# reesque/SfmFromScratch

Measured on AMD Instinct MI355X. Metric: images/sec detect+describe+match, 1080p, 1/2/4/8 MI355X, higher is better.
Workload: dtype f32; 1 GPU; BASELINE configs[1]: 32x 1080p per GPU, ScaleRotInvSIFT 4-level x2 octave pyramid, k=2500, fw 18, NNRatio 0.85 over consecutive pairs; frames_per_gpu=32, pairs_per_gpu=31, distinct_batches=2, parallelism=image-shard x1, batches_in_flight=2

## Files before the change

include/sfmfeat.h:

```cpp
#ifndef SFMFEAT_H_
#define SFMFEAT_H_

#include <stddef.h>
#include <stdint.h>

#ifdef __cplusplus
extern "C" {
#endif

#define SFM_OK 0
#define SFM_EINVAL 1
#define SFM_ESTATE 2
#define SFM_EDEVICE 3
#define SFM_ERANGE 4
#define SFM_EINDEX 5

#define SFM_MODE_SCALEROT 0
#define SFM_MODE_NAIVE 1

#define SFM_DESC_DIM 128
#define SFM_MAX_GAUSS 15
#define SFM_MAX_KSIZE 31
#define SFM_MAX_FW 64
#define SFM_MAX_LEVELS 12
// ... 158 lines not shown
#define SFM_PROF_MEDIAN 2
#define SFM_PROF_NMS 3
#define SFM_PROF_TOPK 4
#define SFM_PROF_DESCRIBE 5
#define SFM_PROF_MATCH_PREP 6
#define SFM_PROF_MATCH 7
#define SFM_PROF_MATCH_POST 8
#define SFM_PROF_STAGES 9
int32_t sfm_profile_enable(sfm_ctx* ctx, int32_t on);
int32_t sfm_profile_stages(sfm_ctx* ctx, int32_t mask);
int32_t sfm_profile_read(sfm_ctx* ctx, double* ms, int64_t* launches, int32_t reset);
int32_t sfm_profile_spans(sfm_ctx* ctx, int64_t capacity);
int32_t sfm_profile_spans_read(sfm_ctx* ctx, int64_t* spans_ns, int32_t* levels, int64_t cap, int64_t* n_out,
                               int64_t* dropped, int32_t reset);

int32_t sfm_debug_atan2(int32_t device, const float* y, const float* x, float* out, int64_t n);
int32_t sfm_debug_harris(int32_t device, const float* gauss, int32_t gs, double alpha,
                         int32_t ksize, const float* img, int32_t H, int32_t W, float* R_out,
                         float* median_out, int64_t* ncand_out);

int32_t sfm_debug_nms(int32_t device, const float* R, int32_t B, int32_t H, int32_t W, int32_t ksize,
                      const uint32_t* tnms, int32_t tile, uint64_t* keys_out, int64_t* counts_out);

float sfm_debug_time_harris(int32_t device, int32_t abl, int32_t B, int32_t H, int32_t W,
                            int32_t iters);
float sfm_debug_harris_stamps(int32_t device, int32_t abl, int32_t B, int32_t H, int32_t W,
                              int32_t iters, uint64_t* out, int64_t cap);

int64_t sfm_debug_match_stamps(uint64_t* out, int64_t cap);

int32_t sfm_copy_wg(void* dst, const void* src, int64_t bytes, int32_t workgroups, void* stream);

int32_t sfm_debug_select_stats(sfm_ctx* ctx, int32_t* fallback_planes, int32_t* total_planes);
int32_t sfm_debug_pose_candidates(sfm_ctx* ctx, int32_t* cand_idx, int64_t entries);
int32_t sfm_debug_copy_level(sfm_ctx* ctx, int32_t l, int32_t what, float* out, void* stream);


#ifdef __cplusplus
}
#endif

#endif
```

sfmfromscratch_amd/_native.py:

```python
from __future__ import annotations

import ctypes
import os
import sys
import threading

import numpy as np

from . import _abi
from ._abi import SfmParams

_HERE = os.path.dirname(os.path.abspath(__file__))
LIB_PATH = os.environ.get("SFMFEAT_LIB", os.path.join(_HERE, "lib", "libsfmfeat.so"))

_lib = None
_lib_lock = threading.Lock()

_fp = ctypes.POINTER(ctypes.c_float)
_i64p = ctypes.POINTER(ctypes.c_int64)
_i32p = ctypes.POINTER(ctypes.c_int32)
_u8p = ctypes.POINTER(ctypes.c_uint8)
_dp = ctypes.POINTER(ctypes.c_double)
_vp = ctypes.c_void_p

# ... 68 lines not shown
    "sfm_profile_read": (ctypes.c_int32, [_vp, ctypes.POINTER(ctypes.c_double), _i64p, ctypes.c_int32]),
    "sfm_profile_spans": (ctypes.c_int32, [_vp, ctypes.c_int64]),
    "sfm_profile_spans_read": (ctypes.c_int32, [_vp, _i64p, _i32p, ctypes.c_int64, _i64p, _i64p, ctypes.c_int32]),
    "sfm_debug_time_harris": (ctypes.c_float, [ctypes.c_int32] * 6),
    "sfm_debug_harris_stamps": (ctypes.c_float, [ctypes.c_int32] * 6 + [ctypes.c_void_p, ctypes.c_int64]),
    "sfm_debug_match_stamps": (ctypes.c_int64, [ctypes.c_void_p, ctypes.c_int64]),
    "sfm_debug_select_stats": (ctypes.c_int32, [_vp, _i32p, _i32p]),
    "sfm_copy_wg": (ctypes.c_int32, [_vp, _vp, ctypes.c_int64, ctypes.c_int32, _vp]),
    "sfm_dist_unique_id": (ctypes.c_int32, [_u8p]),
    "sfm_dist_create": (ctypes.c_int32, [ctypes.c_int32, ctypes.c_int32, ctypes.c_int32, _u8p, ctypes.POINTER(_vp)]),
    "sfm_dist_destroy": (ctypes.c_int32, [_vp]),
    "sfm_dist_last_error": (ctypes.c_char_p, [_vp]),
    "sfm_dist_rank": (ctypes.c_int32, [_vp, _i32p, _i32p]),
    "sfm_dist_allgather_slots_dev": (ctypes.c_int32, [_vp, ctypes.c_int32, ctypes.c_int32, _vp, _vp, _vp, _vp, _vp,
                                                      _vp, ctypes.c_int64, _vp]),
    "sfm_dist_halo_dev": (ctypes.c_int32, [_vp, ctypes.c_int32, _vp, _vp, _vp, _vp, _vp, _vp, _vp]),

    "sfm_debug_copy_level": (ctypes.c_int32, [_vp, ctypes.c_int32, ctypes.c_int32, _vp, _vp]),
    "sfm_debug_atan2": (ctypes.c_int32, [ctypes.c_int32, _fp, _fp, _fp, ctypes.c_int64]),
    "sfm_debug_harris": (ctypes.c_int32, [ctypes.c_int32, _fp, ctypes.c_int32, ctypes.c_double, ctypes.c_int32,
                                          _fp, ctypes.c_int32, ctypes.c_int32, _fp, _fp, _i64p]),
    "sfm_debug_nms": (ctypes.c_int32, [ctypes.c_int32, _fp, ctypes.c_int32, ctypes.c_int32, ctypes.c_int32,
                                       ctypes.c_int32, _vp, ctypes.c_int32, _vp, _i64p]),
}


class NativeLibraryMissing(ImportError):
    pass


def _preload_torch_hip_runtime():
    import importlib.util
    spec = importlib.util.find_spec("torch")
    if spec is None or not spec.submodule_search_locations:
        return
    for d in spec.submodule_search_locations:
        cand = os.path.join(d, "lib", "libamdhip64.so")
        if os.path.exists(cand):
            try:
                ctypes.CDLL(cand, mode=ctypes.RTLD_GLOBAL)
            except OSError:
                pass
            return


def _preload_torch_rccl():
# ... 281 lines not shown
    H, W = img.shape
    gs = int(params.gaussian_size)
    g = np.array(params.gauss_kernel[: gs * gs], np.float32)
    R = np.empty_like(img)
    med = np.zeros(1, np.float32)
    nc = ctypes.c_int64(0)
    check(load_library().sfm_debug_harris(device, g.ctypes.data_as(_fp), gs, params.alpha, params.ksize,
                                          img.ctypes.data_as(_fp), H, W, R.ctypes.data_as(_fp),
                                          med.ctypes.data_as(_fp), ctypes.byref(nc)))
    return R, med[0], nc.value


def debug_nms(R: np.ndarray, tnms, ksize: int = 3, tile: bool = False, device: int = 0):
    R = np.ascontiguousarray(R, dtype=np.float32)
    B, H, W = R.shape
    t = np.ascontiguousarray(tnms, dtype=np.uint32)
    keys = np.zeros(B * H * W, np.uint64)
    cnt = np.zeros(B, np.int64)
    check(load_library().sfm_debug_nms(device, R.ctypes.data_as(_fp), B, H, W, ksize, t.ctypes.data,
                                       int(tile), keys.ctypes.data, cnt.ctypes.data_as(_i64p)))
    return [np.sort(keys[b * H * W: b * H * W + cnt[b]]) for b in range(B)]


class Gate:

    def __init__(self, device: int = 0):
        self.lib = load_library()
        h = _vp()
        if self.lib.sfm_gate_create(device, ctypes.byref(h)) != _abi.SFM_OK:
            raise RuntimeError("sfm_gate_create failed: no usable MI355X (HIP) device")
        self.handle = h

    def attach(self, ctx: Context):
        check(self.lib.sfm_ctx_set_gate(ctx.handle, self.handle), ctx.handle)

    def close(self):
        if getattr(self, "handle", None) is not None and self.handle.value:
            self.lib.sfm_gate_destroy(self.handle)
            self.handle = _vp()

    def __del__(self):
        try:
            self.close()
        except Exception:
            pass

# ... 85 lines not shown
```

sfmfromscratch_amd/csrc/api_extract.hip:

```cpp
#include "ctx.h"

using namespace sfm;

static_assert(kLayoutMedBins == kMedBins1 && kLayoutCounterStride == kCounterStride &&
                  kLayoutMedianStateBytes == sizeof(MedianState) && kLayoutSelectMaxLevels == kSelectMaxLevels,
              "extract_layout.h mirrors kernels.h");

const ExtractSwitches& extract_switches() {
  static const ExtractSwitches sw = [] {
    ExtractSwitches s;
    s.layout.pyr_fused = env_int(getenv("SFMFEAT_PYR_FUSED"), 1) != 0;
    s.layout.exact_px = env_int(getenv("SFMFEAT_EXACT_PX"), 128);
    s.layout.select_merge = env_int(SFM_DIAG_ENV("SFMFEAT_SELECT_MERGE"), 1) != 0;
    s.fill_launches = env_int(SFM_DIAG_ENV("SFMFEAT_FILL_LAUNCHES"), 0) != 0;
    s.harris_group = env_int(SFM_DIAG_ENV("SFMFEAT_HARRIS_GROUP"), 0);
    s.gate_level = env_int(SFM_DIAG_ENV("SFMFEAT_GATE_LEVEL"), 0);
    s.select_caller = env_int(SFM_DIAG_ENV("SFMFEAT_SELECT_CALLER"), 0) == 1;
    s.skip = env_int(SFM_ABLATION_ENV("SFMFEAT_SKIP"), 0);
    return s;
  }();
  return sw;
}

namespace {
// ... 104 lines not shown
    g.n = y.L - y.L_aux;
    for (int l = y.L_aux; l < y.L; ++l)
      g.l[l - y.L_aux] = SelectLevels::Level{R(l), cand(l), candcnt + y.counter[l], at<uint32_t>(kBufMedlist, y.sel[l]),
                                             at<uint64_t>(kBufScratch, y.sel[l]), kp(l), med(l), y.lv[l].h, y.lv[l].w,
                                             y.lv[l].fw / 2};
    if (!(skip & 1)) launch_select_levels(g, std::max(c->kcap, 1), c->kcap, B, c->p.ksize, st);
  }

  void describe_level(int l, hipStream_t s) {
    StageScope sc(c, SFM_PROF_DESCRIBE, s);
    const int L = y.L;
    if ((skip & 2) && l != L - 1) {
      fused_ok = false;
      return;
    }
    bool ow = false;
    const bool r = launch_describe(lvl[l], B, y.lv[l].h, y.lv[l].w, y.lv[l].fw, c->p.mode == SFM_MODE_NAIVE ? 0 : 1,
                                   kp(l), c->kcap, as<int32_t>(c->ex.buf[kBufLc]), l, L, y.lv[l].scale, xy, desc, conf,
                                   cap, l == L - 1 ? count : nullptr, mo, &ow, s);
    if (l == L - 1) counted = r;
    fused_ok = fused_ok && ow;
  }

  int release_gate() {
    if (c->gate && !gate_released) {
      HIPCHK(c, hipEventRecord(c->gate->ev, st));
      c->gate->armed = true;
      gate_released = true;
    }
    return SFM_OK;
  }

  int run(const float* imgs);
};

int Extraction::run(const float* imgs) {
  const int L = y.L, L_aux = y.L_aux;
  CtxStreams& cs = c->s;
  int rc;
  lvl[0] = imgs;
  for (int l = 1; l < L; ++l) lvl[l] = at<float>(kBufLvl, y.lvl[l]);
  zeroed = sw.fill_launches;
  {
    StageScope sc(c, SFM_PROF_PYRAMID, st);
    if (!y.pyr_fused) pyramid_from(1);
  }
// ... 27 lines not shown
    for (int l = l0; l < l1; ++l) {
      if (!exact(l)) {
        StageScope sc(c, SFM_PROF_NMS, st);
        launch_nms(R(l), med(l), cand(l), candcnt + y.counter[l], B, y.lv[l].h, y.lv[l].w, c->p.ksize, 0, st);
      }
      if (l < L_aux) {
        if (sw.select_caller) select_level(l, st);
        HIPCHK(c, hipEventRecord(cs.ev[l], st));
        HIPCHK(c, hipStreamWaitEvent(ax, cs.ev[l], 0));
        if (!sw.select_caller) select_level(l, ax);
        if (l == L_aux - 1) HIPCHK(c, hipEventRecord(cs.ev[L + 2], ax));
        describe_level(l, ax);
      }
    }
    l0 = l1;
  }
  if ((rc = release_gate())) return rc;
  if (y.select_merged) {
    select_merged();
  } else {
    for (int l = L_aux; l < L; ++l) select_level(l, st);
  }
  if (L_aux > 0 && L > L_aux) HIPCHK(c, hipStreamWaitEvent(st, cs.ev[L + 2], 0));
  for (int l = L_aux; l < L; ++l) describe_level(l, st);
  if (L_aux > 0) {
    HIPCHK(c, hipEventRecord(cs.ev[L + 1], ax));
    HIPCHK(c, hipStreamWaitEvent(st, cs.ev[L + 1], 0));
  }
  if (!counted) launch_finalize_counts(as<int32_t>(c->ex.buf[kBufLc]), B, L, count, st);
  HIPCHK(c, hipGetLastError());
  if (fused_ok && counted) operands_fused_commit(c, B);
  return SFM_OK;
}

}

int extract_reserve(sfm_ctx* c, int B, int H, int W) {
  ExtractLayout y;
  if (int rc = layout_of(c, B, H, W, &y)) return rc;
  return reserve(c, y);
}

int extract_impl(sfm_ctx* c, const float* imgs, int B, int H, int W, int32_t* xy, float* desc, float* conf,
                 int32_t* count, int64_t cap, hipStream_t st) {
  if (B < 1 || H < 1 || W < 1) return set_err(c, SFM_EINVAL, "empty batch or image");
  if (cap < c->cap) return set_err(c, SFM_ERANGE, "slot capacity below L * int(k / L)");
  ExtractLayout y;
// ... 88 lines not shown
```

sfmfromscratch_amd/csrc/debug.hip:

```cpp
#include <string.h>

#include <vector>

#include "../../include/sfmfeat.h"
#include "kernels.h"

using namespace sfm;

namespace sfm {

__global__ void k_debug_atan2(const float* __restrict__ y, const float* __restrict__ x,
                              float* __restrict__ out, int64_t n) {
  int64_t i = (int64_t)blockIdx.x * blockDim.x + threadIdx.x;
  if (i < n) out[i] = svml_atan2f(y[i], x[i]);
}

__global__ void __launch_bounds__(256) k_copy_wg(const uint4* __restrict__ src, uint4* __restrict__ dst, int64_t n16,
                                                 const uint8_t* __restrict__ src_b, uint8_t* __restrict__ dst_b,
                                                 int64_t tail) {
  const int64_t stride = (int64_t)gridDim.x * blockDim.x;
  for (int64_t i = (int64_t)blockIdx.x * blockDim.x + threadIdx.x; i < n16; i += stride) dst[i] = src[i];
  if (blockIdx.x == 0 && threadIdx.x < tail) dst_b[threadIdx.x] = src_b[threadIdx.x];
}

// ... 78 lines not shown
      hipMalloc(&d_cnt, 8 * (size_t)B * kCounterStride) || hipMalloc(&d_cand, tot * 8)) {
    rc = SFM_EDEVICE;
  } else {
    std::vector<MedianState> ms(B);
    memset(ms.data(), 0, sizeof(MedianState) * B);
    for (int b = 0; b < B; ++b) ms[b].tnms = tnms[b];
    (void)hipMemcpy(d_R, R, tot * 4, hipMemcpyHostToDevice);
    (void)hipMemcpy(d_med, ms.data(), sizeof(MedianState) * B, hipMemcpyHostToDevice);
    (void)hipMemset(d_cnt, 0, 8 * (size_t)B * kCounterStride);
    launch_nms(d_R, d_med, d_cand, d_cnt, B, H, W, ksize, 0, 0, tile);
    std::vector<unsigned long long> cnt((size_t)B * kCounterStride);
    if (hipDeviceSynchronize() || hipMemcpy(cnt.data(), d_cnt, 8 * cnt.size(), hipMemcpyDeviceToHost) ||
        hipMemcpy(keys_out, d_cand, tot * 8, hipMemcpyDeviceToHost)) {
      rc = SFM_EDEVICE;
    } else {
      for (int b = 0; b < B; ++b) counts_out[b] = (int64_t)cnt[(size_t)b * kCounterStride];
    }
  }
  void* bufs[] = {d_R, d_med, d_cnt, d_cand};
  for (void* b : bufs) (void)hipFree(b);
  return rc;
}

float sfm_debug_time_harris(int32_t device, int32_t abl, int32_t B, int32_t H, int32_t W, int32_t iters) {
  return sfm_debug_harris_stamps(device, abl, B, H, W, iters, nullptr, 0);
}

float sfm_debug_harris_stamps(int32_t device, int32_t abl, int32_t B, int32_t H, int32_t W, int32_t iters,
                              uint64_t* out, int64_t cap) {
  if (hipSetDevice(device) != hipSuccess) return -1.0f;
  uint64_t* d_st = nullptr;
  if (abl == 3) {
    if (cap <= 0 || hipMalloc(&d_st, (size_t)cap * 8) != hipSuccess) return -1.0f;
    (void)hipMemset(d_st, 0, (size_t)cap * 8);
  }
  int64_t n = (int64_t)B * H * W;
  float *d_img = nullptr, *d_R = nullptr, *d_g = nullptr;
  uint32_t* d_hist = nullptr;
  if (hipMalloc(&d_img, n * 4) || hipMalloc(&d_R, n * 4) || hipMalloc(&d_g, 4 * harris_taps_floats(7)) ||
      hipMalloc(&d_hist, (size_t)B * 4 * kMedBins1))
    return -1.0f;
  std::vector<float> h(n);
  uint32_t x = 12345u;
  for (int64_t i = 0; i < n; ++i) {
    x = x * 1664525u + 1013904223u;
    h[i] = (float)(x >> 24) / 255.0f;
// ... 33 lines not shown
```

sfmfromscratch_amd/csrc/describe.hip:

```cpp
#include "kernels.h"

#include <stdlib.h>

namespace sfm {

SFM_DEV double pi_edge(int i, int num) {
  const double start = -3.141592653589793, stop = 3.141592653589793;
  if (i == num - 1) return stop;
  double step = (stop - start) / (double)(num - 1);
  return (double)i * step + start;
}

struct DescLayout {
  int ws, n, n4, pw, P;
  size_t off_keys, off_patch, off_ori, off_mag, off_sw, off_cw, off_cellw, off_wgh, total;
};

__host__ __device__ inline DescLayout desc_layout(int fw, int rotate) {
  DescLayout L;
  int h = fw / 2;
  L.ws = 2 * h;
  L.n = L.ws * L.ws;
  L.pw = L.ws + 2;
  int P = 1;
// ... 238 lines not shown
  if (lane == 0) {
    if (out_conf) out_conf[slot] = kp.conf[ko];
    out_xy[slot * 2 + 0] = (int32_t)((double)x * scale);
    out_xy[slot * 2 + 1] = (int32_t)((double)y * scale);
  }
}

__global__ void k_finalize_counts(const int32_t* __restrict__ lc_all, int B, int L,
                                  int32_t* __restrict__ out_count) {
  int b = blockIdx.x * blockDim.x + threadIdx.x;
  if (b >= B) return;
  int32_t s = 0;
  for (int l = 0; l < L; ++l) s += lc_all[(int64_t)l * B + b];
  out_count[b] = s;
}

size_t describe_lds_bytes(int fw, int rotate) { return desc_layout(fw, rotate).total; }

void init_describe_attributes(size_t max_lds) {
  (void)hipFuncSetAttribute((const void*)k_describe, hipFuncAttributeMaxDynamicSharedMemorySize,
                            (int)max_lds);
}

bool launch_describe(const float* lvl, int B, int H, int W, int fw, int rotate, KpList kp,
                     int kcap, const int32_t* level_counts_all, int level, int L, double scale,
                     int32_t* out_xy, float* out_desc, float* out_conf, int64_t out_cap,
                     int32_t* out_count, const MatchOperands& mo, bool* operands_written, hipStream_t st) {
  if (operands_written) *operands_written = false;
  if (kcap <= 0) return false;
  static const bool one_per_wave = [] {
    const char* v = getenv("SFMFEAT_DESCRIBE");
    return v && v[0] == 'w';
  }();
  if (!one_per_wave && launch_describe_quad(lvl, B, H, W, fw, rotate, kp, kcap, level_counts_all, level,
                                            scale, out_xy, out_desc, out_conf, out_cap, out_count, L, mo, st)) {
    if (operands_written) *operands_written = mo.hi != nullptr;
    return out_count != nullptr;
  }
  size_t lds = describe_lds_bytes(fw, rotate);
  hipLaunchKernelGGL(k_describe, dim3(kcap, B), dim3(64), lds, st, lvl, H, W, fw, rotate, kp, kcap,
                     level_counts_all, level, B, scale, out_xy, out_desc, out_conf, out_cap);
  return false;
}

void launch_finalize_counts(const int32_t* level_counts_all, int B, int L, int32_t* out_count,
                            hipStream_t st) {
  hipLaunchKernelGGL(k_finalize_counts, dim3((B + 255) / 256), dim3(256), 0, st, level_counts_all, B, L,
                     out_count);
}

}
```

sfmfromscratch_amd/csrc/describe_q.hip:

```cpp
#include "kernels.h"

#include <stdlib.h>
#include <string.h>

#include <mutex>

namespace sfm {
namespace dq {

constexpr int cmax(int a, int b) { return a > b ? a : b; }
constexpr int pow2ceil(int v) { return v <= 1 ? 1 : 2 * pow2ceil((v + 1) / 2); }

template <int WS, int ROT>
struct Geo {
  static constexpr int N = WS * WS, PW = WS + 2, NP = PW * PW;
  static constexpr int P = cmax(pow2ceil(N), 16), E = P / 16;
  static constexpr int RN = (N + 15) / 16;
  static constexpr int A = (cmax(cmax(NP, N + 4), 16 * 17) + 3) & ~3;
  static constexpr int NQ = (N + 3) & ~3;
  static constexpr int OFF_M = A;
  static constexpr int OFF_K = OFF_M + NQ;
  static constexpr int OFF_R = OFF_K + NQ;
  static constexpr int OFF_I = OFF_R + (ROT ? (NQ / 2 + 3) & ~3 : 0);
  static constexpr int OFF_T = OFF_I + (ROT ? 40 : 0);
// ... 57 lines not shown
  b = hi;
}
SFM_DEV double keep_or_take(bool lower, double mine, double other) {
  const double lo = __builtin_fmin(mine, other), hi = __builtin_fmax(mine, other);
  return lower ? lo : hi;
}

template <int E, int S>
SFM_DEV void half_clean(double (&k)[E], int gl) {
  if constexpr (S >= 1) {
    if constexpr (S < E) {
#pragma unroll
      for (int r = 0; r < E; ++r)
        if ((r & S) == 0) cas_up(k[r], k[r + S]);
    } else {
      constexpr int X = S / E;
      const bool lower = (gl & X) == 0;
#pragma unroll
      for (int r = 0; r < E; ++r) k[r] = keep_or_take(lower, k[r], rxord<X>(k[r]));
    }
    half_clean<E, S / 2>(k, gl);
  }
}
template <int E, int SIZE>
SFM_DEV void merge_level(double (&k)[E], int gl) {
  if constexpr (SIZE <= 16 * E) {
    if constexpr (SIZE <= E) {
#pragma unroll
      for (int r = 0; r < E; ++r)
        if ((r & (SIZE / 2)) == 0) cas_up(k[r], k[r ^ (SIZE - 1)]);
    } else {
      constexpr int X = SIZE / E - 1;
      const bool lower = (gl & ((X + 1) >> 1)) == 0;
      if constexpr (E == 1) {
        k[0] = keep_or_take(lower, k[0], rxord<X>(k[0]));
      } else {
#pragma unroll
        for (int r = 0; r < E / 2; ++r) {
          const double oa = rxord<X>(k[E - 1 - r]);
          const double ob = rxord<X>(k[r]);
          k[r] = keep_or_take(lower, k[r], oa);
          k[E - 1 - r] = keep_or_take(lower, k[E - 1 - r], ob);
        }
      }
    }
    half_clean<E, SIZE / 4>(k, gl);
    merge_level<E, SIZE * 2>(k, gl);
  }
}

SFM_DEV void grad_at(const float* c, int pw, float& mag, float& ori) {
  const float a00 = c[-pw - 1], a01 = c[-pw], a02 = c[-pw + 1];
  const float a10 = c[-1], a12 = c[1];
  const float a20 = c[pw - 1], a21 = c[pw], a22 = c[pw + 1];
  float gx = 0.0f;
  gx = __builtin_fmaf(-1.0f, a00, gx);
  gx = __builtin_fmaf(1.0f, a02, gx);
  gx = __builtin_fmaf(-2.0f, a10, gx);
  gx = __builtin_fmaf(2.0f, a12, gx);
  gx = __builtin_fmaf(-1.0f, a20, gx);
  gx = __builtin_fmaf(1.0f, a22, gx);
  float gy = 0.0f;
  gy = __builtin_fmaf(-1.0f, a00, gy);
  gy = __builtin_fmaf(-2.0f, a01, gy);
  gy = __builtin_fmaf(-1.0f, a02, gy);
  gy = __builtin_fmaf(1.0f, a20, gy);
  gy = __builtin_fmaf(2.0f, a21, gy);
  gy = __builtin_fmaf(1.0f, a22, gy);
  const float sx = gx * gx;
  const float sy = gy * gy;
// ... 370 lines not shown
    }
    *reinterpret_cast<h8*>(mo.hi + mr * 128 + gl * 8) = hh;
    *reinterpret_cast<h8*>(mo.lo + mr * 128 + gl * 8) = ll;
    s += rxord<8>(s);
    s += rxord<4>(s);
    s += rxord<2>(s);
    s += rxord<1>(s);
    if (gl == 0) {
      const float n2 = (float)s, rn = (float)sqrt(s);
      mo.norm2[mr] = n2;
      mo.rnorm[mr] = rn;
      float2* pm = mo.pmax + (int64_t)b * (mo.capP / kPrepRows) + r / kPrepRows;
      atomicMax(reinterpret_cast<unsigned int*>(&pm->x), __float_as_uint(n2));
      atomicMax(reinterpret_cast<unsigned int*>(&pm->y), __float_as_uint(rn));
    }
  }
  if (gl == 0) {
    if (out_conf) out_conf[slot] = kp.conf[ko];
    out_xy[slot * 2 + 0] = (int32_t)((double)x * scale);
    out_xy[slot * 2 + 1] = (int32_t)((double)y * scale);
  }
}

}

namespace {
uint32_t fkey_h(float v) {
  uint32_t b;
  memcpy(&b, &v, 4);
  if (b == 0x80000000u) b = 0u;
  return (b & 0x80000000u) ? ~b : (b | 0x80000000u);
}
float fkey_inv_h(uint32_t k) {
  const uint32_t b = (k & 0x80000000u) ? (k & 0x7fffffffu) : ~k;
  float f;
  memcpy(&f, &b, 4);
  return f;
}
double pi_edge_h(int i, int num) {
  const double start = -3.141592653589793, stop = 3.141592653589793;
  if (i == num - 1) return stop;
  const double step = (stop - start) / (double)(num - 1);
  return (double)i * step + start;
}
uint32_t edge_key_h(double e, double sh, bool strict) {
  uint32_t kc = fkey_h((float)(e + sh));
// ... 4 lines not shown
  for (int it = 0; it < 64 && pass(kc); ++it) --kc;
  for (int it = 0; it < 64 && !pass(kc); ++it) ++kc;
  return kc;
}
}

void init_describe_quad_tables() {
  static std::mutex mu;
  static bool done[256] = {};
  int dev = 0;
  if (hipGetDevice(&dev) != hipSuccess || dev < 0 || dev >= 256) return;
  std::lock_guard<std::mutex> lk(mu);
  if (done[dev]) return;
  uint32_t ori[37], cell[37][9];
  for (int j = 0; j < 37; ++j) ori[j] = edge_key_h(pi_edge_h(j, 37), 0.0, j == 36);
  for (int bi = 0; bi < 37; ++bi) {
    const double dom = bi < 36 ? (pi_edge_h(bi, 37) + pi_edge_h(bi + 1, 37)) / 2.0 : 0.0;
    for (int t = 0; t < 9; ++t) cell[bi][t] = edge_key_h(pi_edge_h(t, 9), dom, t == 8);
  }
  done[dev] = hipMemcpyToSymbol(HIP_SYMBOL(dq::c_ori), ori, sizeof(ori)) == hipSuccess &&
              hipMemcpyToSymbol(HIP_SYMBOL(dq::c_cell), cell, sizeof(cell)) == hipSuccess;
}

#define SFM_DQ_BODY(WS)                                                                              \
    if (rotate)                                                                                      \
      hipLaunchKernelGGL((dq::k_describe_q<WS, 1>), grid, dim3(64), 0, st, lvl, H, W, kp, kcap, lc,  \
                         level, B, scale, out_xy, out_desc, out_conf, out_cap, out_count, L, mo);        \
    else                                                                                             \
      hipLaunchKernelGGL((dq::k_describe_q<WS, 0>), grid, dim3(64), 0, st, lvl, H, W, kp, kcap, lc,  \
                         level, B, scale, out_xy, out_desc, out_conf, out_cap, out_count, L, mo);        \
    return true;
#define SFM_DQ_CASE(WS) \
  case WS:              \
    SFM_DQ_BODY(WS)

bool launch_describe_quad(const float* lvl, int B, int H, int W, int fw, int rotate, KpList kp, int kcap,
                          const int32_t* lc, int level, double scale, int32_t* out_xy, float* out_desc,
                          float* out_conf, int64_t out_cap, int32_t* out_count, int L, const MatchOperands& mo,
                          hipStream_t st) {
  constexpr int kPadBlocks = 8;
  const dim3 grid((kcap + 3) / 4 + (mo.hi != nullptr && out_count != nullptr ? kPadBlocks : 0), B);
  switch (2 * (fw / 2)) {
    SFM_DQ_CASE(2)
    SFM_DQ_CASE(4)
    SFM_DQ_CASE(6)
    SFM_DQ_CASE(8)
    SFM_DQ_CASE(10)
// ... 41 lines not shown
```

sfmfromscratch_amd/csrc/kernels.h:

```cpp
#pragma once

#include <hip/hip_runtime.h>
#include <stdint.h>

#include <vector>

#include "common.h"

namespace sfm {

#define SFM_NMS_MAX_HALF 15

constexpr int kHistBits = 12;
constexpr int kHistBins = 1 << kHistBits;
constexpr int kMedBits1 = 11;
constexpr int kMedBins1 = 1 << kMedBits1;
constexpr int kTopkLdsCap = 8192;
constexpr int kMaxMatchRows = 16384;
constexpr int kMatchCandCap = 256;
constexpr int kCounterStride = 32;
constexpr int kMatchUnitPairBits = 20;

constexpr float kMatchScale = 256.0f;
constexpr float kMatchLoScale = 2048.0f;
// ... 288 lines not shown
void launch_select(const float* R, uint64_t* cand, const unsigned long long* cand_count, uint32_t* medlist,
                   uint64_t* scratch, KpList kp, int kcap, int k, int B, int H, int W, int ksize, int half_window,
                   MedianState* state, hipStream_t st);
constexpr int kSelectMaxLevels = 4;
struct SelectLevels {
  struct Level {
    const float* R;
    uint64_t* cand;
    const unsigned long long* cand_count;
    uint32_t* medlist;
    uint64_t* scratch;
    KpList kp;
    MedianState* state;
    int H, W, hw;
  } l[kSelectMaxLevels];
  int n;
};
void launch_select_levels(const SelectLevels& g, int kcap, int k, int B, int ksize, hipStream_t st);

bool launch_describe_quad(const float* lvl, int B, int H, int W, int fw, int rotate, KpList kp, int kcap,
                          const int32_t* level_counts_all, int level, double scale, int32_t* out_xy,
                          float* out_desc, float* out_conf, int64_t out_cap, int32_t* out_count, int L,
                          const MatchOperands& mo, hipStream_t st);
bool launch_describe(const float* lvl, int B, int H, int W, int fw, int rotate, KpList kp,
                     int kcap, const int32_t* level_counts_all, int level, int L, double scale,
                     int32_t* out_xy, float* out_desc, float* out_conf, int64_t out_cap,
                     int32_t* out_count, const MatchOperands& mo, bool* operands_written, hipStream_t st);
void launch_finalize_counts(const int32_t* level_counts_all, int B, int L, int32_t* out_count,
                            hipStream_t st);

struct RowBest {
  int32_t col;
  float nndr;
};
void launch_transpose_desc(const float* desc, const int32_t* count, int nimg, int64_t cap,
                           int64_t capP, float* descT, hipStream_t st);
void launch_match_rows(const float* descT, const int32_t* count, int64_t capP, const int32_t* pairs,
                       int P, float ratio, RowBest* rows, int max_rows, hipStream_t st);
void launch_match_compact(const RowBest* rows, const int32_t* count, const int32_t* pairs, int P,
                          int max_rows, int64_t cap, int32_t* matches, float* conf, int32_t* nmatch,
                          int* reset_counter, hipStream_t st);
void init_match_attributes(int max_rows);
size_t match_pmax_bytes(int64_t capP);
void launch_match_prep(const float* desc, const int32_t* count, int nimg, int64_t cap, int64_t capP,
                       _Float16* hi, _Float16* lo, float* norm2, float* rnorm, void* pmax, hipStream_t st);
void launch_match_mfma(const float* desc, const int32_t* count, int64_t cap, int64_t capP,
// ... 7 lines not shown
```

Baseline: 42900 images/sec.

## Pack multiple keypoints per wave and batch describe levels into one launch

Adds a packed describe kernel that assigns 8 or 16 keypoints to a single 64-lane wave, using 4 or 8 lanes per keypoint, for small window sizes. It also merges up to four pyramid levels' describe work into one launch through a level table with per-level workgroup offsets. The aim is to reduce idle lanes and per-level launch overhead in the describe stage. In exchange it brings in a large new kernel with its own sort, prefix and histogram paths, and adds a debug describe entry point.

```diff
diff --git a/include/sfmfeat.h b/include/sfmfeat.h
--- a/include/sfmfeat.h
+++ b/include/sfmfeat.h
@@ -204,6 +204,9 @@
 int32_t sfm_debug_nms(int32_t device, const float* R, int32_t B, int32_t H, int32_t W, int32_t ksize,
                       const uint32_t* tnms, int32_t tile, uint64_t* keys_out, int64_t* counts_out);
 
+int32_t sfm_debug_describe(int32_t device, const float* img, int32_t H, int32_t W, const int32_t* x,
+                           const int32_t* y, int32_t n, int32_t fw, int32_t rotate, float* desc_out);
+
 float sfm_debug_time_harris(int32_t device, int32_t abl, int32_t B, int32_t H, int32_t W,
                             int32_t iters);
 float sfm_debug_harris_stamps(int32_t device, int32_t abl, int32_t B, int32_t H, int32_t W,
diff --git a/sfmfromscratch_amd/_native.py b/sfmfromscratch_amd/_native.py
--- a/sfmfromscratch_amd/_native.py
+++ b/sfmfromscratch_amd/_native.py
@@ -114,6 +114,8 @@
                                           _fp, ctypes.c_int32, ctypes.c_int32, _fp, _fp, _i64p]),
     "sfm_debug_nms": (ctypes.c_int32, [ctypes.c_int32, _fp, ctypes.c_int32, ctypes.c_int32, ctypes.c_int32,
                                        ctypes.c_int32, _vp, ctypes.c_int32, _vp, _i64p]),
+    "sfm_debug_describe": (ctypes.c_int32, [ctypes.c_int32, _fp, ctypes.c_int32, ctypes.c_int32, _i32p, _i32p,
+                                            ctypes.c_int32, ctypes.c_int32, ctypes.c_int32, _fp]),
 }
 
 
@@ -441,6 +443,20 @@
     return [np.sort(keys[b * H * W: b * H * W + cnt[b]]) for b in range(B)]
 
 
+def debug_describe(img: np.ndarray, x, y, fw: int, rotate: bool = True, device: int = 0) -> np.ndarray:
+    img = np.ascontiguousarray(img, dtype=np.float32)
+    H, W = img.shape
+    x = np.ascontiguousarray(x, dtype=np.int32)
+    y = np.ascontiguousarray(y, dtype=np.int32)
+    if x.shape != y.shape or x.ndim != 1:
+        raise ValueError("x and y must be 1-D arrays of one length")
+    out = np.zeros((x.size, 128), np.float32)
+    check(load_library().sfm_debug_describe(device, img.ctypes.data_as(_fp), H, W, x.ctypes.data_as(_i32p),
+                                            y.ctypes.data_as(_i32p), x.size, int(fw), int(bool(rotate)),
+                                            out.ctypes.data_as(_fp)))
+    return out
+
+
 class Gate:
 
     def __init__(self, device: int = 0):
diff --git a/sfmfromscratch_amd/csrc/api_extract.hip b/sfmfromscratch_amd/csrc/api_extract.hip
--- a/sfmfromscratch_amd/csrc/api_extract.hip
+++ b/sfmfromscratch_amd/csrc/api_extract.hip
@@ -150,6 +150,33 @@
     fused_ok = fused_ok && ow;
   }
 
+  void describe_run(int l0, int l1, hipStream_t s) {
+    StageScope sc(c, SFM_PROF_DESCRIBE, s);
+    const int L = y.L;
+    DescribeLevels g{};
+    g.n = l1 - l0;
+    for (int l = l0; l < l1; ++l)
+      g.l[l - l0] = DescribeLevels::Level{lvl[l], kp(l), y.lv[l].scale, y.lv[l].h, y.lv[l].w, 2 * (y.lv[l].fw / 2),
+                                          l, 0, 0};
+    launch_describe_levels(g, B, c->p.mode == SFM_MODE_NAIVE ? 0 : 1, c->kcap, as<int32_t>(c->ex.buf[kBufLc]), xy,
+                           desc, conf, cap, l1 == L ? count : nullptr, L, mo, s);
+    if (l1 == L) counted = true;
+    fused_ok = fused_ok && mo.hi != nullptr;
+  }
+
+  void describe_tail(int l0, hipStream_t s) {
+    const int L = y.L;
+    int r0 = L;
+    if (!describe_one_per_wave() && !(skip & 2) && c->kcap > 0)
+      while (r0 > l0 && describe_packs(y.lv[r0 - 1].fw)) --r0;
+    for (int l = l0; l < r0; ++l) describe_level(l, s);
+    for (int l = r0; l < L;) {
+      const int n = (L - l) % kDescribeMaxLevels ? (L - l) % kDescribeMaxLevels : kDescribeMaxLevels;
+      describe_run(l, l + n, s);
+      l += n;
+    }
+  }
+
   int release_gate() {
     if (c->gate && !gate_released) {
       HIPCHK(c, hipEventRecord(c->gate->ev, st));
@@ -223,7 +250,7 @@
     for (int l = L_aux; l < L; ++l) select_level(l, st);
   }
   if (L_aux > 0 && L > L_aux) HIPCHK(c, hipStreamWaitEvent(st, cs.ev[L + 2], 0));
-  for (int l = L_aux; l < L; ++l) describe_level(l, st);
+  describe_tail(L_aux, st);
   if (L_aux > 0) {
     HIPCHK(c, hipEventRecord(cs.ev[L + 1], ax));
     HIPCHK(c, hipStreamWaitEvent(st, cs.ev[L + 1], 0));
diff --git a/sfmfromscratch_amd/csrc/debug.hip b/sfmfromscratch_amd/csrc/debug.hip
--- a/sfmfromscratch_amd/csrc/debug.hip
+++ b/sfmfromscratch_amd/csrc/debug.hip
@@ -124,6 +124,40 @@
   return rc;
 }
 
+int32_t sfm_debug_describe(int32_t device, const float* img, int32_t H, int32_t W, const int32_t* x,
+                           const int32_t* y, int32_t n, int32_t fw, int32_t rotate, float* desc_out) {
+  if (H < 1 || W < 1 || n < 0 || fw < 1 || fw > SFM_MAX_FW || !img || (n > 0 && (!x || !y || !desc_out)))
+    return SFM_EINVAL;
+  if (n == 0) return SFM_OK;
+  if (hipSetDevice(device) != hipSuccess) return SFM_EDEVICE;
+  init_describe_attributes(describe_lds_bytes(SFM_MAX_FW, 1));
+  init_describe_quad_tables();
+  const size_t px = (size_t)H * W;
+  float *d_img = nullptr, *d_conf = nullptr, *d_desc = nullptr;
+  int32_t *d_x = nullptr, *d_y = nullptr, *d_cnt = nullptr, *d_xy = nullptr;
+  int32_t rc = SFM_OK;
+  if (hipMalloc(&d_img, px * 4) || hipMalloc(&d_conf, (size_t)n * 4) || hipMalloc(&d_desc, (size_t)n * 128 * 4) ||
+      hipMalloc(&d_x, (size_t)n * 4) || hipMalloc(&d_y, (size_t)n * 4) || hipMalloc(&d_cnt, 4) ||
+      hipMalloc(&d_xy, (size_t)n * 8)) {
+    rc = SFM_EDEVICE;
+  } else {
+    (void)hipMemcpy(d_img, img, px * 4, hipMemcpyHostToDevice);
+    (void)hipMemcpy(d_x, x, (size_t)n * 4, hipMemcpyHostToDevice);
+    (void)hipMemcpy(d_y, y, (size_t)n * 4, hipMemcpyHostToDevice);
+    (void)hipMemcpy(d_cnt, &n, 4, hipMemcpyHostToDevice);
+    (void)hipMemset(d_conf, 0, (size_t)n * 4);
+    (void)hipMemset(d_desc, 0xFF, (size_t)n * 128 * 4);
+    launch_describe(d_img, 1, H, W, fw, rotate ? 1 : 0, KpList{d_x, d_y, d_conf, d_cnt}, n, d_cnt, 0, 1, 1.0, d_xy,
+                    d_desc, nullptr, n, nullptr, MatchOperands{nullptr, nullptr, nullptr, nullptr, nullptr, 0}, nullptr,
+                    0);
+    if (hipDeviceSynchronize() || hipMemcpy(desc_out, d_desc, (size_t)n * 128 * 4, hipMemcpyDeviceToHost))
+      rc = SFM_EDEVICE;
+  }
+  void* bufs[] = {d_img, d_conf, d_desc, d_x, d_y, d_cnt, d_xy};
+  for (void* b : bufs) (void)hipFree(b);
+  return rc;
+}
+
 float sfm_debug_time_harris(int32_t device, int32_t abl, int32_t B, int32_t H, int32_t W, int32_t iters) {
   return sfm_debug_harris_stamps(device, abl, B, H, W, iters, nullptr, 0);
 }
diff --git a/sfmfromscratch_amd/csrc/describe.hip b/sfmfromscratch_amd/csrc/describe.hip
--- a/sfmfromscratch_amd/csrc/describe.hip
+++ b/sfmfromscratch_amd/csrc/describe.hip
@@ -284,16 +284,30 @@
                             (int)max_lds);
 }
 
+bool describe_one_per_wave() {
+  static const bool one_per_wave = [] {
+    const char* v = getenv("SFMFEAT_DESCRIBE");
+    return v && v[0] == 'w';
+  }();
+  return one_per_wave;
+}
+
 bool launch_describe(const float* lvl, int B, int H, int W, int fw, int rotate, KpList kp,
                      int kcap, const int32_t* level_counts_all, int level, int L, double scale,
                      int32_t* out_xy, float* out_desc, float* out_conf, int64_t out_cap,
                      int32_t* out_count, const MatchOperands& mo, bool* operands_written, hipStream_t st) {
   if (operands_written) *operands_written = false;
   if (kcap <= 0) return false;
-  static const bool one_per_wave = [] {
-    const char* v = getenv("SFMFEAT_DESCRIBE");
-    return v && v[0] == 'w';
-  }();
+  const bool one_per_wave = describe_one_per_wave();
+  if (!one_per_wave && describe_packs(fw)) {
+    DescribeLevels g{};
+    g.n = 1;
+    g.l[0] = DescribeLevels::Level{lvl, kp, scale, H, W, 2 * (fw / 2), level, 0, 0};
+    launch_describe_levels(g, B, rotate, kcap, level_counts_all, out_xy, out_desc, out_conf, out_cap, out_count,
+                           L, mo, st);
+    if (operands_written) *operands_written = mo.hi != nullptr;
+    return out_count != nullptr;
+  }
   if (!one_per_wave && launch_describe_quad(lvl, B, H, W, fw, rotate, kp, kcap, level_counts_all, level,
                                             scale, out_xy, out_desc, out_conf, out_cap, out_count, L, mo, st)) {
     if (operands_written) *operands_written = mo.hi != nullptr;
diff --git a/sfmfromscratch_amd/csrc/describe_q.hip b/sfmfromscratch_amd/csrc/describe_q.hip
--- a/sfmfromscratch_amd/csrc/describe_q.hip
+++ b/sfmfromscratch_amd/csrc/describe_q.hip
@@ -103,9 +103,9 @@
     half_clean<E, S / 2>(k, gl);
   }
 }
-template <int E, int SIZE>
+template <int E, int SIZE, int LANES = 16>
 SFM_DEV void merge_level(double (&k)[E], int gl) {
-  if constexpr (SIZE <= 16 * E) {
+  if constexpr (SIZE <= LANES * E) {
     if constexpr (SIZE <= E) {
 #pragma unroll
       for (int r = 0; r < E; ++r)
@@ -126,7 +126,7 @@
       }
     }
     half_clean<E, SIZE / 4>(k, gl);
-    merge_level<E, SIZE * 2>(k, gl);
+    merge_level<E, SIZE * 2, LANES>(k, gl);
   }
 }
 
@@ -543,6 +543,427 @@
   }
 }
 
+template <int WS, int ROT>
+struct GeoP {
+  static constexpr int N = WS * WS, PW = WS + 2, NP = PW * PW;
+  static constexpr int LPK = WS <= 4 ? 4 : 8, KPW = 64 / LPK;
+  static constexpr int NC = WS <= 4 ? 1 : 4;
+  static constexpr int P = cmax(pow2ceil(N), LPK), E = P / LPK;
+  static constexpr int RN = (N + LPK - 1) / LPK;
+  static constexpr int A = (cmax(cmax(NP, N + 4), NC * 17) + 3) & ~3;
+  static constexpr int NQ = (N + 3) & ~3;
+  static constexpr int OFF_M = A;
+  static constexpr int OFF_K = OFF_M + NQ;
+  static constexpr int OFF_R = OFF_K + NQ;
+  static constexpr int OFF_I = OFF_R + (ROT ? (NQ / 2 + 3) & ~3 : 0);
+  static constexpr int OFF_T = OFF_I + (ROT ? 40 : 0);
+  static constexpr int G = OFF_T + 12;
+  static constexpr int LDS = KPW * G;
+  static_assert(RN <= E && (N + E - 1) / E <= LPK, "pixels fit the sort slots; the prefix chain fits the lanes");
+};
+template <int ROT>
+constexpr int packed_lds_floats() {
+  return cmax(cmax(GeoP<2, ROT>::LDS, GeoP<4, ROT>::LDS), cmax(GeoP<6, ROT>::LDS, GeoP<8, ROT>::LDS));
+}
+
+template <int WS, int ROT>
+SFM_DEV void describe_packed(const DescribeLevels::Level& lv, int wg, int b, float* s_all, int kcap,
+                             const int32_t* __restrict__ lc_all, int B, int32_t* __restrict__ out_xy,
+                             float* __restrict__ out_desc, float* __restrict__ out_conf, int64_t out_cap,
+                             const MatchOperands& mo) {
+  using C = GeoP<WS, ROT>;
+  constexpr int N = C::N, PW = C::PW, NP = C::NP, E = C::E, RN = C::RN, h = WS / 2;
+  constexpr int LPK = C::LPK, KPW = C::KPW, NC = C::NC;
+  const int H = lv.H, W = lv.W;
+  const KpList& kp = lv.kp;
+  const int count = kp.count[b];
+  const int kbase = wg * KPW;
+  if (kbase >= count) return;
+  const int lane = threadIdx.x, g = lane / LPK, gl = lane & (LPK - 1);
+  const int kpi = kbase + g;
+  const bool valid = kpi < count;
+  const int64_t ko = (int64_t)b * kcap + (valid ? kpi : kbase);
+  const int x = kp.x[ko], y = kp.y[ko];
+  float* sA = s_all + g * C::G;
+  float* sM = sA + C::OFF_M;
+  uint32_t* sK = reinterpret_cast<uint32_t*>(sA + C::OFF_K);
+  uint16_t* sR = reinterpret_cast<uint16_t*>(sA + C::OFF_R);
+  int32_t* sI = reinterpret_cast<int32_t*>(sA + C::OFF_I);
+  uint32_t* sT = reinterpret_cast<uint32_t*>(sA + C::OFF_T);
+
+  const float* img = lv.lvl + (int64_t)b * H * W;
+#pragma unroll
+  for (int it = 0; it < (NP + LPK - 1) / LPK; ++it) {
+    const int e0 = it * LPK + gl;
+    const int e = e0 < NP ? e0 : NP - 1;
+    const int pr = e / PW, pc = e - pr * PW;
+    const int gy = y - h + pr, gx = x - h + pc;
+    const bool in = gy >= 0 && gy < H && gx >= 0 && gx < W;
+    const int cy = min(max(gy, 0), H - 1), cx = min(max(gx, 0), W - 1);
+    const float v = img[(int64_t)cy * W + cx];
+    if (e0 < NP) sA[e] = in ? v : 0.0f;
+  }
+  __syncthreads();
+
+  double k[E];
+  bool tiny = false;
+#pragma unroll
+  for (int r = 0; r < E; ++r) k[r] = __longlong_as_double((long long)kPad);
+#pragma unroll
+  for (int r = 0; r < RN; ++r) {
+    const int e0 = r * LPK + gl;
+    const bool ok = (N % LPK == 0) || e0 < N;
+    const int e = ok ? e0 : N - 1;
+    const int i = e / WS, j = e - i * WS;
+    float mag, ori;
+    grad_at(sA + (i + 1) * PW + (j + 1), PW, mag, ori);
+    if (ok) {
+      sM[e] = mag;
+      if (!ROT) sK[e] = __float_as_uint(ori);
+    }
+    if (ROT) {
+      k[r] = ok ? dkey(((uint64_t)fkey(ori) << 9) | (uint32_t)e) : __longlong_as_double((long long)kPad);
+      tiny |= ok && ori != 0.0f && fabsf(ori) < 0x1p-25f;
+    }
+  }
+  __syncthreads();
+
+  int dom_bin = 36;
+  double dom = 0.0;
+  if constexpr (ROT) {
+    merge_level<E, 2, LPK>(k, gl);
+    float w[E];
+    uint32_t ke[E], kf[E];
+#pragma unroll
+    for (int r = 0; r < E; ++r) {
+      const int p = gl * E + r;
+      const uint64_t pl = dpayload(k[r]);
+      ke[r] = p < N ? (uint32_t)(pl & 511u) : 0u;
+      kf[r] = (uint32_t)(pl >> 9);
+      w[r] = p < N ? sM[ke[r]] : 0.0f;
+    }
+    __syncthreads();
+    float cw[E];
+#pragma unroll
+    for (int r = 0; r < E; ++r) cw[r] = 0.0f;
+    float carry = 0.0f;
+    constexpr int NL = (N + E - 1) / E;
+#pragma unroll
+    for (int s = 0; s < NL; ++s) {
+      if (gl == s) {
+        float acc = carry;
+#pragma unroll
+        for (int r = 0; r < E; ++r) {
+          acc = acc + w[r];
+          cw[r] = acc;
+        }
+      }
+      const float nxt = __uint_as_float(dpp<0x111>(__float_as_uint(cw[E - 1])));
+      if (gl == s + 1) carry = nxt;
+    }
+#pragma unroll
+    for (int r = 0; r < E; r += (E >= 4 ? 4 : 1)) {
+      const int p = gl * E + r;
+      if (p < N) {
+        if constexpr (E >= 4) {
+          *reinterpret_cast<uint4*>(sK + p) = make_uint4(kf[r], kf[r + 1], kf[r + 2], kf[r + 3]);
+          *reinterpret_cast<float4*>(sM + p) = make_float4(w[r], w[r + 1], w[r + 2], w[r + 3]);
+          *reinterpret_cast<float4*>(sA + 4 + p) = make_float4(cw[r], cw[r + 1], cw[r + 2], cw[r + 3]);
+        } else {
+          sK[p] = kf[r];
+          sM[p] = w[r];
+          sA[4 + p] = cw[r];
+        }
+      }
+    }
+#pragma unroll
+    for (int r = 0; r < E; ++r) {
+      const int p = gl * E + r;
+      if (p < N) sR[ke[r]] = (uint16_t)p;
+    }
+    if (gl == 0) sA[3] = 0.0f;
+    __syncthreads();
+#pragma unroll
+    for (int t = 0; t < (37 + LPK - 1) / LPK; ++t) {
+      const int j = gl + LPK * t;
+      if (j <= 36) {
+        const uint32_t T = c_ori[j];
+        int lo = 0;
+        constexpr int S0 = pow2ceil(N + 1) / 2;
+#pragma unroll
+        for (int s = S0; s >= 1; s >>= 1) {
+          const int q = lo + s;
+          const uint32_t v = sK[(q <= N ? q : N) - 1];
+          if (q <= N && v < T) lo = q;
+        }
+        sI[j] = lo;
+      }
+    }
+    __syncthreads();
+    float hb = -INFINITY;
+    int bi = 64;
+#pragma unroll
+    for (int t = 0; t < (36 + LPK - 1) / LPK; ++t) {
+      const int j = gl + LPK * t;
+      if (j < 36) {
+        const float v = sA[3 + sI[j + 1]] - sA[3 + sI[j]];
+        if (v > hb) { hb = v; bi = j; }
+      }
+    }
+    {
+      float ov; int oi;
+      if constexpr (LPK == 8) {
+        ov = rxorf<4>(hb); oi = (int)rxor<4>((uint32_t)bi);
+        if (ov > hb || (ov == hb && oi < bi)) { hb = ov; bi = oi; }
+      }
+      ov = rxorf<2>(hb); oi = (int)rxor<2>((uint32_t)bi);
+      if (ov > hb || (ov == hb && oi < bi)) { hb = ov; bi = oi; }
+      ov = rxorf<1>(hb); oi = (int)rxor<1>((uint32_t)bi);
+      if (ov > hb || (ov == hb && oi < bi)) { hb = ov; bi = oi; }
+    }
+    dom = (pi_edge(bi, 37) + pi_edge(bi + 1, 37)) / 2.0;
+    dom_bin = bi;
+  }
+
+#pragma unroll
+  for (int t = 0; t < (9 + LPK - 1) / LPK; ++t)
+    if (gl + LPK * t < 9) sT[gl + LPK * t] = c_cell[dom_bin][gl + LPK * t];
+  __syncthreads();
+  const bool cell_ok = gl < NC;
+  const int r4 = NC == 1 ? 0 : (gl >> 1) & 1, c4 = NC == 1 ? 0 : gl & 1;
+  float hv[8];
+  float wv[16];
+  uint32_t hk[16];
+  const bool grp_tiny = ROT && ((__ballot(tiny) >> (LPK * g)) & ((1ull << LPK) - 1)) != 0;
+  if (ROT && !grp_tiny) {
+    uint32_t q[16];
+    if constexpr (NC == 1) {
+#pragma unroll
+      for (int t = 0; t < 16; ++t) q[t] = cell_ok && t < N ? (uint32_t)t : 0xFFFFFFFFu;
+    } else {
+#pragma unroll
+      for (int t = 0; t < 16; ++t) {
+        const int i = 4 * r4 + (t >> 2), j = 4 * c4 + (t & 3);
+        const bool ok = cell_ok && i < WS && j < WS;
+        q[t] = ok ? (uint32_t)sR[ok ? i * WS + j : 0] : 0xFFFFFFFFu;
+      }
+      batcher16(q);
+    }
+#pragma unroll
+    for (int m = 0; m < 16; ++m) {
+      const bool ok = q[m] != 0xFFFFFFFFu;
+      const uint32_t p = ok ? q[m] : 0u;
+      wv[m] = ok ? sM[p] : 0.0f;
+      hk[m] = ok ? sK[p] : 0xFFFFFFFFu;
+    }
+  } else {
+    uint64_t q[16];
+#pragma unroll
+    for (int t = 0; t < 16; ++t) {
+      const int i = 4 * r4 + (t >> 2), j = 4 * c4 + (t & 3);
+      const bool ok = cell_ok && i < WS && j < WS;
+      const int e = ok ? i * WS + j : 0;
+      const uint32_t key = ROT ? sK[sR[e]] : fkey(__uint_as_float(sK[e]));
+      q[t] = ok ? (((uint64_t)key << 32) | (uint32_t)t) : ~0ull;
+    }
+    if (!ROT) {
+      double dq16[16];
+#pragma unroll
+      for (int t = 0; t < 16; ++t) dq16[t] = q[t] == ~0ull ? __longlong_as_double((long long)kPad)
+                                                           : dkey(((q[t] >> 32) << 4) | (uint32_t)t);
+      batcher16(dq16);
+#pragma unroll
+      for (int t = 0; t < 16; ++t) {
+        const uint64_t pl = dpayload(dq16[t]);
+        q[t] = pl >= (1ull << 36) ? ~0ull : (((pl >> 4) << 32) | (pl & 15u));
+      }
+    } else {
+      double cv[16];
+      int sl[16];
+#pragma unroll
+      for (int t = 0; t < 16; ++t) {
+        cv[t] = q[t] == ~0ull ? INFINITY : (double)fkey_inv((uint32_t)(q[t] >> 32)) - dom;
+        sl[t] = t;
+      }
+#pragma unroll
+      for (int p = 1; p < 16; p <<= 1)
+#pragma unroll
+        for (int kk = p; kk >= 1; kk >>= 1)
+#pragma unroll
+          for (int j = kk % p; j + kk < 16; j += 2 * kk)
+#pragma unroll
+            for (int i = 0; i < kk; ++i) {
+              const int a = i + j, c = i + j + kk;
+              if (c < 16 && a / (2 * p) == c / (2 * p)) {
+                const bool sw = cv[a] > cv[c] || (cv[a] == cv[c] && sl[a] > sl[c]);
+                const double tv = cv[a];
+                cv[a] = sw ? cv[c] : tv;
+                cv[c] = sw ? tv : cv[c];
+                const uint64_t tq = q[a];
+                q[a] = sw ? q[c] : tq;
+                q[c] = sw ? tq : q[c];
+                const int ts = sl[a];
+                sl[a] = sw ? sl[c] : ts;
+                sl[c] = sw ? ts : sl[c];
+              }
+            }
+    }
+#pragma unroll
+    for (int m = 0; m < 16; ++m) {
+      const bool ok = q[m] != ~0ull;
+      const int t = ok ? (int)(uint32_t)q[m] : 0;
+      const int e = ok ? (4 * r4 + (t >> 2)) * WS + 4 * c4 + (t & 3) : 0;
+      wv[m] = ok ? (ROT ? sM[sR[e]] : sM[e]) : 0.0f;
+      hk[m] = ok ? (uint32_t)(q[m] >> 32) : 0xFFFFFFFFu;
+    }
+  }
+  float* cc = sA + (cell_ok ? gl : 0) * 17;
+  float acc = 0.0f;
+  if (cell_ok) cc[0] = 0.0f;
+#pragma unroll
+  for (int m = 0; m < 16; ++m) {
+    acc = acc + wv[m];
+    if (cell_ok) cc[m + 1] = acc;
+  }
+  int bidx[9];
+#pragma unroll
+  for (int eb = 0; eb < 9; ++eb) {
+    const uint32_t T = sT[eb];
+    int c = 0;
+#pragma unroll
+    for (int m = 0; m < 16; ++m) c += hk[m] < T ? 1 : 0;
+    bidx[eb] = c;
+  }
+#pragma unroll
+  for (int bb = 0; bb < 8; ++bb) hv[bb] = cc[bidx[bb + 1]] - cc[bidx[bb]];
+
+  float tr[8];
+#pragma unroll
+  for (int t = 0; t < 8; ++t) tr[t] = hv[t] * hv[t];
+  if constexpr (NC == 4) {
+#pragma unroll
+    for (int t = 0; t < 8; ++t) tr[t] = tr[t] + rxorf<2>(tr[t]);
+#pragma unroll
+    for (int t = 0; t < 8; ++t) tr[t] = tr[t] + rxorf<1>(tr[t]);
+  }
+#pragma unroll
+  for (int t = 0; t < 4; ++t) tr[t] = tr[t] + tr[t + 4];
+  tr[0] = tr[0] + tr[2];
+  tr[1] = tr[1] + tr[3];
+  tr[0] = tr[0] + tr[1];
+  const float nrm = sqrtf(tr[0]);
+  if (!valid) return;
+  int64_t off0 = 0;
+  for (int l = 0; l < lv.level; ++l) off0 += lc_all[(int64_t)l * B + b];
+  const int64_t slot = (int64_t)b * out_cap + off0 + kpi;
+  const int cell = 4 * r4 + c4;
+  auto live = [](int c) { return NC == 1 ? c == 0 : (c & ~5) == 0; };
+  float o[8];
+#pragma unroll
+  for (int t = 0; t < 8; ++t) o[t] = sqrtf(nrm > 0.0f ? hv[t] / nrm : hv[t]);
+  float4* row = reinterpret_cast<float4*>(out_desc + slot * 128);
+  if (cell_ok) {
+    row[2 * cell] = make_float4(o[0], o[1], o[2], o[3]);
+    row[2 * cell + 1] = make_float4(o[4], o[5], o[6], o[7]);
+  }
+#pragma unroll
+  for (int it = 0; it < 32 / LPK; ++it) {
+    const int f = gl + LPK * it;
+    if (!live(f >> 1)) row[f] = make_float4(0.0f, 0.0f, 0.0f, 0.0f);
+  }
+  if (mo.hi != nullptr) {
+    const int64_t r = off0 + kpi, mr = (int64_t)b * mo.capP + r;
+    typedef _Float16 h8 __attribute__((ext_vector_type(8)));
+    h8 hh, ll;
+    double s = 0.0;
+#pragma unroll
+    for (int t = 0; t < 8; ++t) {
+      const float xs = o[t] * kMatchScale;
+      const _Float16 hv16 = (_Float16)xs;
+      const float rr = (xs - (float)hv16) * kMatchLoScale;
+      hh[t] = hv16;
+      ll[t] = (_Float16)rr;
+      s += (double)o[t] * (double)o[t];
+    }
+    uint4* hrow = reinterpret_cast<uint4*>(mo.hi + mr * 128);
+    uint4* lrow = reinterpret_cast<uint4*>(mo.lo + mr * 128);
+    if (cell_ok) {
+      *reinterpret_cast<h8*>(hrow + cell) = hh;
+      *reinterpret_cast<h8*>(lrow + cell) = ll;
+    }
+#pragma unroll
+    for (int it = 0; it < 16 / LPK; ++it) {
+      const int c = gl + LPK * it;
+      if (!live(c)) {
+        hrow[c] = make_uint4(0u, 0u, 0u, 0u);
+        lrow[c] = make_uint4(0u, 0u, 0u, 0u);
+      }
+    }
+    if constexpr (NC == 4) {
+      s += rxord<2>(s);
+      s += rxord<1>(s);
+    }
+    if (gl == 0) {
+      const float n2 = (float)s, rn = (float)sqrt(s);
+      mo.norm2[mr] = n2;
+      mo.rnorm[mr] = rn;
+      float2* pm = mo.pmax + (int64_t)b * (mo.capP / kPrepRows) + r / kPrepRows;
+      atomicMax(reinterpret_cast<unsigned int*>(&pm->x), __float_as_uint(n2));
+      atomicMax(reinterpret_cast<unsigned int*>(&pm->y), __float_as_uint(rn));
+    }
+  }
+  if (gl == 0) {
+    if (out_conf) out_conf[slot] = kp.conf[ko];
+    out_xy[slot * 2 + 0] = (int32_t)((double)x * lv.scale);
+    out_xy[slot * 2 + 1] = (int32_t)((double)y * lv.scale);
+  }
+}
+
+template <int ROT>
+__global__ void __launch_bounds__(64) k_describe_qp(DescribeLevels g, int kcap, const int32_t* __restrict__ lc_all,
+                                                    int B, int32_t* __restrict__ out_xy,
+                                                    float* __restrict__ out_desc, float* __restrict__ out_conf,
+                                                    int64_t out_cap, int32_t* __restrict__ out_count, int L,
+                                                    MatchOperands mo) {
+  __shared__ __attribute__((aligned(16))) float s_all[packed_lds_floats<ROT>()];
+  const int b = blockIdx.y;
+  if (out_count != nullptr && blockIdx.x == 0 && threadIdx.x == 0) {
+    int32_t s = 0;
+    for (int l = 0; l < L; ++l) s += lc_all[(int64_t)l * B + b];
+    out_count[b] = s;
+  }
+  if ((int)blockIdx.x >= g.nwg) {
+    int32_t s = 0;
+    for (int l = 0; l < L; ++l) s += lc_all[(int64_t)l * B + b];
+    const int nt = ((int)gridDim.x - g.nwg) * 64;
+    for (int64_t r = s + ((int)blockIdx.x - g.nwg) * 64 + threadIdx.x; r < mo.capP; r += nt) {
+      const int64_t mr = (int64_t)b * mo.capP + r;
+      uint4* hz = reinterpret_cast<uint4*>(mo.hi + mr * 128);
+      uint4* lz = reinterpret_cast<uint4*>(mo.lo + mr * 128);
+#pragma unroll
+      for (int q = 0; q < 16; ++q) {
+        hz[q] = make_uint4(0u, 0u, 0u, 0u);
+        lz[q] = make_uint4(0u, 0u, 0u, 0u);
+      }
+      mo.norm2[mr] = INFINITY;
+      mo.rnorm[mr] = 0.0f;
+    }
+    return;
+  }
+  int li = 0;
+  for (int i = 1; i < g.n; ++i)
+    if ((int)blockIdx.x >= g.l[i].wg0) li = i;
+  const DescribeLevels::Level& lv = g.l[li];
+  const int wg = (int)blockIdx.x - lv.wg0;
+  switch (lv.ws) {
+    case 2: describe_packed<2, ROT>(lv, wg, b, s_all, kcap, lc_all, B, out_xy, out_desc, out_conf, out_cap, mo); break;
+    case 4: describe_packed<4, ROT>(lv, wg, b, s_all, kcap, lc_all, B, out_xy, out_desc, out_conf, out_cap, mo); break;
+    case 6: describe_packed<6, ROT>(lv, wg, b, s_all, kcap, lc_all, B, out_xy, out_desc, out_conf, out_cap, mo); break;
+    case 8: describe_packed<8, ROT>(lv, wg, b, s_all, kcap, lc_all, B, out_xy, out_desc, out_conf, out_cap, mo); break;
+    default: break;
+  }
+}
+
 }
 
 namespace {
@@ -593,7 +1014,34 @@
               hipMemcpyToSymbol(HIP_SYMBOL(dq::c_cell), cell, sizeof(cell)) == hipSuccess;
 }
 
-#define SFM_DQ_BODY(WS)                                                                              \
+bool describe_packs(int fw) {
+  static const bool on = env_int(SFM_DIAG_ENV("SFMFEAT_DESCRIBE_PACK"), 1) != 0;
+  const int ws = 2 * (fw / 2);
+  return on && ws >= 2 && ws <= 8;
+}
+
+void launch_describe_levels(DescribeLevels g, int B, int rotate, int kcap, const int32_t* lc, int32_t* out_xy,
+                            float* out_desc, float* out_conf, int64_t out_cap, int32_t* out_count, int L,
+                            const MatchOperands& mo, hipStream_t st) {
+  constexpr int kPadBlocks = 8;
+  int wg = 0;
+  for (int i = 0; i < g.n; ++i) {
+    const int kpw = g.l[i].ws <= 4 ? 16 : 8;
+    g.l[i].wg0 = wg;
+    g.l[i].nwg = (kcap + kpw - 1) / kpw;
+    wg += g.l[i].nwg;
+  }
+  g.nwg = wg;
+  const dim3 grid(wg + (mo.hi != nullptr && out_count != nullptr ? kPadBlocks : 0), B);
+  if (rotate)
+    hipLaunchKernelGGL((dq::k_describe_qp<1>), grid, dim3(64), 0, st, g, kcap, lc, B, out_xy, out_desc, out_conf,
+                       out_cap, out_count, L, mo);
+  else
+    hipLaunchKernelGGL((dq::k_describe_qp<0>), grid, dim3(64), 0, st, g, kcap, lc, B, out_xy, out_desc, out_conf,
+                       out_cap, out_count, L, mo);
+}
+
+#define SFM_DQ_BODY(WS)                                                                             \
     if (rotate)                                                                                      \
       hipLaunchKernelGGL((dq::k_describe_q<WS, 1>), grid, dim3(64), 0, st, lvl, H, W, kp, kcap, lc,  \
                          level, B, scale, out_xy, out_desc, out_conf, out_cap, out_count, L, mo);        \
diff --git a/sfmfromscratch_amd/csrc/kernels.h b/sfmfromscratch_amd/csrc/kernels.h
--- a/sfmfromscratch_amd/csrc/kernels.h
+++ b/sfmfromscratch_amd/csrc/kernels.h
@@ -334,6 +334,22 @@
                           const int32_t* level_counts_all, int level, double scale, int32_t* out_xy,
                           float* out_desc, float* out_conf, int64_t out_cap, int32_t* out_count, int L,
                           const MatchOperands& mo, hipStream_t st);
+constexpr int kDescribeMaxLevels = 4;
+struct DescribeLevels {
+  struct Level {
+    const float* lvl;
+    KpList kp;
+    double scale;
+    int H, W, ws, level, wg0, nwg;
+  } l[kDescribeMaxLevels];
+  int n;
+  int nwg;
+};
+bool describe_packs(int fw);
+void launch_describe_levels(DescribeLevels g, int B, int rotate, int kcap, const int32_t* level_counts_all,
+                            int32_t* out_xy, float* out_desc, float* out_conf, int64_t out_cap,
+                            int32_t* out_count, int L, const MatchOperands& mo, hipStream_t st);
+bool describe_one_per_wave();
 bool launch_describe(const float* lvl, int B, int H, int W, int fw, int rotate, KpList kp,
                      int kcap, const int32_t* level_counts_all, int level, int L, double scale,
                      int32_t* out_xy, float* out_desc, float* out_conf, int64_t out_cap,
```

Result: no change. 43300 images/sec (median of 6 runs) (+0.9%).
